# jsourati/nn-active-learning

Hardware: AMD Instinct MI355X
Metric: patches/sec Fisher-scored (32^3, 2-class) (higher is better)
Workload: dtype f32 (fp32 operands split into 16-bit pieces on the 16-bit MFMA, fp32 accumulate: fp16 pairs - 22-23 bits kept per operand, three products - in the conv under the head (forward + backward), in dec1's forward launch and in the other backward launches; bf16 triples - all 24 bits, exact, six products -

## Files before the change

### nn-active-learning_amd/csrc/alq_internal.h

```cpp
#pragma once
#include <hip/hip_runtime.h>

#include <cstdint>
#include <cstdio>
#include <memory>
#include <string>
#include <vector>

#include "alq.h"

namespace alq {

void set_error(const char *fmt, ...);

#define ALQ_HIP(expr)                                                                     \
    do {                                                                                  \
        hipError_t e_ = (expr);                                                           \
        if (e_ != hipSuccess) {                                                           \
            ::alq::set_error("%s:%d: %s -> %s", __FILE__, __LINE__, #expr,               \
                             hipGetErrorString(e_));                                      \
            return ALQ_EHIP;                                                              \
        }                                                                                 \
    } while (0)

// ... 182 lines not shown
    int *d_tdesc = nullptr, *d_sdesc = nullptr;
};

struct Igemm2Fuse {
    const float *mask = nullptr;
    int mask_cs = 0, mask_c0 = 0, mask_from = 0;
    int mask_to = 1 << 30;
    float *osumA = nullptr, *osumB = nullptr;
    int split = 0;
    int store_from = 0;
    int mask_split = 0;
    long long mask_delta = 0;
    const unsigned char *mask_bits = nullptr;
    unsigned char *sign_out = nullptr;
    const unsigned *in_bits = nullptr;
    const float *in_vec = nullptr;
    float in_vec_amax = 0.f;
    const unsigned *in_vec16 = nullptr;
    unsigned *out_amax = nullptr;
    int amax_from = 0;
    const unsigned *in_amax = nullptr, *in_amax2 = nullptr;
    float in_bound = 0.f;
    const float *fc_W = nullptr;
    long long fc_F = 0;
    float *fc_part = nullptr;
    unsigned *fc_bits = nullptr;
    unsigned *flip_cnt = nullptr, *flip_list = nullptr;
    int flip_cap = 0;
    float flip_l1 = 0.f;
    bool flip_bias_nonzero = false;
};

extern unsigned long long *g_igemm2_dbg;
constexpr int ALQ_NKNOBS = 9;
extern int g_dbg_knobs[ALQ_NKNOBS];
extern int g_dcp_last_form;
extern int g_no_f16x2;
extern int g_no_fixed;
extern int g_no_xcd_order;
int igemm2_build_plan(const IgemmPlan &p1, Igemm2Plan *p2);
void igemm2_pack_weights(Igemm2Plan *p2, const std::vector<float> &Bmat);
int igemm2_launch(alq_ctx *ctx, const Igemm2Plan &plan, const View &in, const View &out, const float *bias,
                  int relu, int accumulate, int N, int prof_cls, const Igemm2Fuse *fuse);

struct Igemm3Plan {
    bool ok = false;
    bool wres = false;
    int NTW = 1;
    int wgs_per_cu = 1;
    size_t lds_bytes = 0;
    std::vector<unsigned short> h_W;
    void *d_W = nullptr;
    std::vector<unsigned short> h_W16;
    void *d_W16 = nullptr;
    int w16_exp = 0;
};
int igemm3_build_plan(const Igemm2Plan &p2, Igemm3Plan *p3);
void igemm3_pack_weights(const Igemm2Plan &p2, Igemm3Plan *p3, const std::vector<float> &Bmat);
void igemm3_pack_weights_f16(const Igemm2Plan &p2, Igemm3Plan *p3, const std::vector<float> &Bmat);
int igemm3_launch(alq_ctx *ctx, const Igemm2Plan &p2, const Igemm3Plan &plan, const View &in, const View &out,
                  const float *bias, int relu, int accumulate, int N, int prof_cls, const Igemm2Fuse *fuse);

struct Igemm4Args {
    const float *in;
    float *out;
    const void *W;
    const float *bias;
// ... 103 lines not shown
void c3d_bwd_pack(C3dPlan *plan, const std::vector<float> &Bmat_fwd );
void c3d_presplit_vec(const float *v, long long F, int e, std::vector<unsigned short> *out);
int c3d_bwd_launch(alq_ctx *ctx, const C3dPlan &plan, int N, const unsigned char *bits, const void *vec16, int e_in, const unsigned char *maskA,
                   float *dB, float *sumA, float *sumB, int rows_per_wave = 8);

struct T3dPlan {
    bool ok = false;
    int kind = 0;
    int w_exp = 0;
    double flops_per_patch = 0;
    std::vector<unsigned short> h_W;
    void *d_W = nullptr;
};
int t3d_build(const View &in, const View &out, const int k[3], const int lo[3], const int s[3], T3dPlan *fwd, T3dPlan *bwd);
void t3d_fwd_pack(T3dPlan *plan, const float *W );
void t3d_bwd_pack(T3dPlan *plan, const float *W);
void t3d8_fwd_pack(T3dPlan *plan, const float *W );
void t3d8_bwd_pack(T3dPlan *plan, const float *W );
int t3d8_bwd_launch(alq_ctx *ctx, const T3dPlan &plan, const View &dout, const View &din, int N, float in_bound, const unsigned char *mask_bits, float *dsum);
int t3d_fwd_launch(alq_ctx *ctx, const T3dPlan &plan, const View &in, const View &out, const float *bias, int N, float *osum, unsigned *out_amax);
int t3d_bwd_launch(alq_ctx *ctx, const T3dPlan &plan, const View &dout, const View &din, int N, float in_bound, const unsigned char *mask_bits,
                   float *dsum);

struct E3dPlan {
    bool ok = false;
    int w_exp = 0;
    double flops_per_patch = 0;
    std::vector<unsigned short> h_Whi, h_Wlo;
    void *d_Whi = nullptr, *d_Wlo = nullptr;
};
int e3d_build(const View &in, const View &out, const int k[3], const int lo[3], const int s[3], E3dPlan *plan);
void e3d_pack(E3dPlan *plan, const float *W );
int e3d_bwd_launch(alq_ctx *ctx, const E3dPlan &plan, int N, const float *skip, const float *dpool, const unsigned char *am2, const unsigned char *sg2,
                   const unsigned char *am1, const unsigned char *sg1, float *dsum2, float *dsum1, float in_bound);

struct D3dPlan {
    bool ok = false;
    int w_exp = 0;
    double flops_per_patch = 0;
    std::vector<unsigned short> h_Whi, h_Wlo;
    void *d_Whi = nullptr, *d_Wlo = nullptr;
    std::vector<unsigned short> h_Bhi, h_Blo;
    void *d_Bhi = nullptr, *d_Blo = nullptr;
};
void d3d_bwd_pack(D3dPlan *plan, const float *W);
int d3d_bwd_launch(alq_ctx *ctx, const D3dPlan &plan, int N, const float *dout, float in_bound, float *dinA, float *dinB, float *sumB);
int d3d_build(const View &in, const View &out, const int k[3], const int lo[3], const int s[3], D3dPlan *plan);
void d3d_pack(D3dPlan *plan, const float *W );
int d3d_fwd_launch(alq_ctx *ctx, const D3dPlan &plan, int N, const float *inA, const float *inB, const unsigned *amaxA, const unsigned *amaxB,
                   const float *bias, int relu, float *out, unsigned char *sg, float *osum);

struct F3dPlan {
    bool ok = false;
    int w_exp = 0;
    double flops_per_patch = 0;
    std::vector<unsigned short> h_Whi, h_Wlo;
    void *d_Whi = nullptr, *d_Wlo = nullptr;
};
int f3d_build(const View &in, const View &out, const int k[3], const int lo[3], const int s[3], F3dPlan *plan);
void f3d_pack(F3dPlan *plan, const float *W );
int f3d_fwd_launch(alq_ctx *ctx, const F3dPlan &plan, int N, const float *in, const unsigned *amax, const float *bias, float *out, unsigned char *sg,
                   float *osum, float *pout, unsigned char *parg, float *posum);

struct DirectArgs {
    const float *in;
    float *out;
    const float *W;
// ... 199 lines not shown
```

### nn-active-learning_amd/csrc/e3d.hip

```cpp
#include "alq_internal.h"

#include <algorithm>
#include <cmath>
#include <cstdlib>
#include <cstring>
#include <vector>

namespace alq {

typedef float f32x4 __attribute__((ext_vector_type(4)));
typedef float f32x2 __attribute__((ext_vector_type(2)));
typedef int i32x4 __attribute__((ext_vector_type(4)));
typedef int i32x2 __attribute__((ext_vector_type(2)));
typedef _Float16 f16x8 __attribute__((ext_vector_type(8)));
typedef _Float16 f16x2 __attribute__((ext_vector_type(2)));

struct E3Args {
    const float *skip;
    const float *dpool;
    const unsigned char *am2;
    const unsigned char *sg2;
    const unsigned short *Whi;
    const unsigned short *Wlo;
    const unsigned char *am1;
// ... 192 lines not shown
                        const f16x8 wlo = *reinterpret_cast<const f16x8 *>(wl + ((dz * 3 + dy) * 2 + s) * 1024);
                        const f16x8 whi = wh[dz * 3 + dy][s];
                        cl = __builtin_amdgcn_mfma_f32_16x16x32_f16(wlo, xh, cl, 0, 0, 0);
                        cl = __builtin_amdgcn_mfma_f32_16x16x32_f16(whi, xl, cl, 0, 0, 0);
                        c = __builtin_amdgcn_mfma_f32_16x16x32_f16(whi, xh, c, 0, 0, 0);
                    }
                }
            }
            const float r0 = __builtin_fmaf(cl.x, 0x1p-11f, c.x) * a.inv, r1 = __builtin_fmaf(cl.y, 0x1p-11f, c.y) * a.inv;
            const float r2 = __builtin_fmaf(cl.z, 0x1p-11f, c.z) * a.inv, r3 = __builtin_fmaf(cl.w, 0x1p-11f, c.w) * a.inv;
            unsigned m0 = (unsigned)__builtin_amdgcn_sbfe((int)sg1b, 0, 1), m1 = (unsigned)__builtin_amdgcn_sbfe((int)sg1b, 1, 1);
            unsigned m2 = (unsigned)__builtin_amdgcn_sbfe((int)sg1b, 2, 1), m3 = (unsigned)__builtin_amdgcn_sbfe((int)sg1b, 3, 1);
            asm("" : "+v"(m0), "+v"(m1), "+v"(m2), "+v"(m3));
            const float v0 = __builtin_bit_cast(float, __builtin_bit_cast(unsigned, r0) & m0), v1 = __builtin_bit_cast(float, __builtin_bit_cast(unsigned, r1) & m1);
            const float v2 = __builtin_bit_cast(float, __builtin_bit_cast(unsigned, r2) & m2), v3 = __builtin_bit_cast(float, __builtin_bit_cast(unsigned, r3) & m3);
            float sw[8];
#pragma unroll
            for (int w = 0; w < 8; ++w)
                sw[w] = ((((am1w & 255u) == (unsigned)w) ? v0 : 0.f) + ((((am1w >> 8) & 255u) == (unsigned)w) ? v1 : 0.f)) +
                        (((((am1w >> 16) & 255u) == (unsigned)w) ? v2 : 0.f) + (((am1w >> 24) == (unsigned)w) ? v3 : 0.f));
            f32x4 mine;
            {
                const float g0 = __shfl_xor(hi ? sw[0] : sw[4], 16, 64), g1 = __shfl_xor(hi ? sw[1] : sw[5], 16, 64);
                const float g2 = __shfl_xor(hi ? sw[2] : sw[6], 16, 64), g3 = __shfl_xor(hi ? sw[3] : sw[7], 16, 64);
                mine = f32x4{(hi ? sw[4] : sw[0]) + g0, (hi ? sw[5] : sw[1]) + g1, (hi ? sw[6] : sw[2]) + g2, (hi ? sw[7] : sw[3]) + g3};
            }
            const f32x2 n0 = f32x2{old0.x + mine.x, old0.y + mine.y}, n1 = f32x2{old1.x + mine.z, old1.y + mine.w};
            __builtin_amdgcn_raw_buffer_store_b64(__builtin_bit_cast(i32x2, n0), d1_rsrc, (int)(tv ? e_d1 : E3_OOB), (int)d1row, 0);
            __builtin_amdgcn_raw_buffer_store_b64(__builtin_bit_cast(i32x2, n1), d1_rsrc, (int)(tv ? e_d1 + 128u : E3_OOB), (int)d1row, 0);
        }
    }
}

int e3d_build(const View &in, const View &out, const int k[3], const int lo[3], const int s[3], E3dPlan *plan) {
    plan->ok = false;
    if (getenv("ALQ_NO_E3D")) return ALQ_OK;
    if (!(k[0] == 3 && k[1] == 3 && k[2] == 3 && s[0] == 1 && s[1] == 1 && s[2] == 1 && lo[0] == 1 && lo[1] == 1 && lo[2] == 1)) return ALQ_OK;
    if (!(in.D == 16 && in.H == 16 && in.W == 16 && out.D == 16 && out.H == 16 && out.W == 16 && in.C == 8 && out.C == 16 && in.split == 0 && out.split == 0)) return ALQ_OK;
    plan->flops_per_patch = 2.0 * 27 * 8 * 16 * 4096.0;
    plan->ok = true;
    return ALQ_OK;
}

void e3d_pack(E3dPlan *plan, const float *W) {
    float amax = 0.f;
    for (size_t i = 0; i < (size_t)27 * 8 * 16; ++i) amax = std::max(amax, std::fabs(W[i]));
    int ex = 0;
    if (amax > 0.f) (void)std::frexp(amax, &ex);
    plan->w_exp = 14 - ex;
    plan->h_Whi.assign((size_t)9 * 2 * 64 * 8, 0);
    plan->h_Wlo.assign((size_t)9 * 2 * 64 * 8, 0);
    for (int dz = 0; dz < 3; ++dz)
        for (int dy = 0; dy < 3; ++dy)
            for (int s = 0; s < 2; ++s)
                for (int lane = 0; lane < 64; ++lane) {
                    const int r = lane & 15, kg = lane >> 4, px = r >> 3, ci = r & 7, q = 2 * s + (kg >> 1);
                    const int tz = 2 - dz, ty = 2 - dy, tx = 2 - q + px;
                    for (int c = 0; c < 8; ++c) {
                        const int co = 8 * (kg & 1) + c;
                        const float w = (tx >= 0 && tx <= 2) ? W[((size_t)((tz * 3 + ty) * 3 + tx) * 8 + ci) * 16 + co] : 0.f;
                        const float ws = std::ldexp(w, plan->w_exp);
                        const _Float16 h = (_Float16)ws;
                        const _Float16 l = (_Float16)std::ldexp(ws - (float)h, 11);
                        unsigned short hb, lb;
                        std::memcpy(&hb, &h, 2);
                        std::memcpy(&lb, &l, 2);
                        const size_t o = ((size_t)((dz * 3 + dy) * 2 + s) * 64 + lane) * 8 + c;
                        plan->h_Whi[o] = hb;
                        plan->h_Wlo[o] = lb;
                    }
                }
}

int e3d_bwd_launch(alq_ctx *ctx, const E3dPlan &plan, int N, const float *skip, const float *dpool, const unsigned char *am2, const unsigned char *sg2,
                   const unsigned char *am1, const unsigned char *sg1, float *dsum2, float *dsum1, float in_bound) {
    ALQ_REQUIRE(plan.ok && plan.d_Whi && plan.d_Wlo, ALQ_EINVAL, "e3d: weights not set");
    ALQ_REQUIRE(skip && dpool && am2 && sg2 && am1 && sg1 && dsum2 && dsum1 && in_bound > 0.f, ALQ_EINVAL, "e3d: missing argument");
    ALQ_REQUIRE(N < 4096, ALQ_EUNSUPPORTED, "e3d: 32-bit byte offsets hold fewer than 4096 patches per pass");
    if (N <= 0) return ALQ_OK;
    int ex = 0;
    (void)std::frexp(in_bound, &ex);
    const int e_in = 14 - ex;
    E3Args a;
    a.skip = skip; a.dpool = dpool; a.am2 = am2; a.sg2 = sg2; a.Whi = reinterpret_cast<const unsigned short *>(plan.d_Whi);
    a.Wlo = reinterpret_cast<const unsigned short *>(plan.d_Wlo); a.am1 = am1; a.sg1 = sg1; a.dsum2 = dsum2; a.dsum1 = dsum1;
    a.scale = std::ldexp(1.f, e_in); a.inv = std::ldexp(1.f, -(e_in + plan.w_exp)); a.N = N;
    const int cus = ctx->num_cus;
    long long g = std::min<long long>(2LL * cus, (long long)N * 4);
    g = std::max<long long>(8, (g + 7) / 8 * 8);
    const size_t lds = E3_WLO + E3_STRIP + E3_SINK;
    ALQ_HIP(hipFuncSetAttribute(reinterpret_cast<const void *>(e3d_bwd_kernel), hipFuncAttributeMaxDynamicSharedMemorySize, (int)lds));
    ProfScope ps(ctx, PROF_IGEMM_F16, plan.flops_per_patch * N);
    hipLaunchKernelGGL(e3d_bwd_kernel, dim3((unsigned)g), dim3(256), lds, ctx->stream, a);
    ALQ_HIP(hipGetLastError());
    return ALQ_OK;
}

}
```

### nn-active-learning_amd/csrc/igemm2.hip

```cpp
#include "alq_internal.h"

#include <algorithm>
#include <cmath>
#include <cstring>

namespace alq {

typedef float f32x4 __attribute__((ext_vector_type(4)));
typedef float f32x2 __attribute__((ext_vector_type(2)));

#ifdef ALQ_STAMPS
#define STAMP(var) asm volatile("s_memtime %0\n\ts_waitcnt lgkmcnt(0)" : "=s"(var)::"memory")
#define PHASE_END(idx)                         \
    do {                                       \
        unsigned long long t_now_;             \
        STAMP(t_now_);                         \
        ph[idx] += t_now_ - t_last;            \
        t_last = t_now_;                       \
    } while (0)
#else
#define PHASE_END(idx) do {} while (0)
#endif

constexpr int I2_CBP = 12;
// ... 451 lines not shown
    }
    p2->NTW = p1.NTW;
    p2->wres = wres;
    p2->lds_bytes = lds;
    int max_wgs = 2;
    if (const char *e = getenv("ALQ_MAX_WGS")) max_wgs = atoi(e);
    p2->wgs_per_cu = std::max<int>(1, std::min<int>(max_wgs, (int)((160 * 1024) / (lds + 512))));
    p2->flops_per_patch = p1.flops_per_patch;
    p2->ok = true;
    return ALQ_OK;
}

void igemm2_pack_weights(Igemm2Plan *p2, const std::vector<float> &Bmat) {
    const Igemm2Args &a = p2->a;
    const int NTW = p2->NTW, Ci = a.Ci, Co = a.Co;
    p2->h_W.assign((size_t)a.nchunks * a.ntaps * NTW * 128, 0.f);
    for (int ch = 0; ch < a.nchunks; ++ch)
        for (int tp = 0; tp < a.ntaps; ++tp)
            for (int nt = 0; nt < NTW; ++nt)
                for (int lane = 0; lane < 64; ++lane)
                    for (int s = 0; s < 2; ++s) {
                        const int c = ch * 8 + 2 * (lane >> 4) + s;
                        const int co = nt * 16 + (lane & 15);
                        if (co < Co)
                            p2->h_W[((((size_t)ch * a.ntaps + tp) * NTW + nt) * 64 + lane) * 2 + s] =
                                Bmat[((size_t)tp * Ci + c) * Co + co];
                    }
}

unsigned long long *g_igemm2_dbg = nullptr;
int g_no_f16x2 = 0;
int g_no_xcd_order = 0;
int g_no_fixed = 0;
int g_dbg_knobs[ALQ_NKNOBS] = {0, 0, 0, 0, 0, 0, 0, 0, 0};

template <int NTW, bool WRES, int GEO, bool SUMS>
static int launch2_s(alq_ctx *ctx, const Igemm2Plan &plan, const Igemm2Args &a, unsigned grid) {
    auto kfn = igemm2_kernel<NTW, WRES, GEO, SUMS>;
    if (plan.lds_bytes > 64 * 1024)
        ALQ_HIP(hipFuncSetAttribute(reinterpret_cast<const void *>(kfn), hipFuncAttributeMaxDynamicSharedMemorySize,
                                    (int)plan.lds_bytes));
    hipLaunchKernelGGL(kfn, dim3(grid), dim3(256), plan.lds_bytes, ctx->stream, a);
    ALQ_HIP(hipGetLastError());
    return ALQ_OK;
}

template <int NTW, bool WRES, int GEO>
static int launch2_t(alq_ctx *ctx, const Igemm2Plan &plan, const Igemm2Args &a, unsigned grid) {
    return (a.osumA || a.osumB) ? launch2_s<NTW, WRES, GEO, true>(ctx, plan, a, grid)
                                : launch2_s<NTW, WRES, GEO, false>(ctx, plan, a, grid);
}

int igemm2_launch(alq_ctx *ctx, const Igemm2Plan &plan, const View &in, const View &out, const float *bias, int relu,
                  int accumulate, int N, int prof_cls, const Igemm2Fuse *fuse) {
    Igemm2Args a = plan.a;
    ALQ_REQUIRE(in.C == a.Ci && in.D == a.ID && in.H == a.IH && in.W == a.IW, ALQ_EINVAL,
                "igemm2: input view does not match plan");
    ALQ_REQUIRE(out.C == a.Co && out.D == a.OD && out.H == a.OH && out.W == a.OW, ALQ_EINVAL,
                "igemm2: output view does not match plan");
    ALQ_REQUIRE(plan.d_W != nullptr, ALQ_EINVAL, "igemm2: weights not set");
    ALQ_REQUIRE((long long)N * in.vox() * in.cs < (1LL << 29) && (long long)N * out.vox() * out.cs < (1LL << 29),
                ALQ_EUNSUPPORTED, "igemm2: tensor exceeds the 32-bit byte-offset range (lower the batch)");
    ALQ_REQUIRE(in.cs % 4 == 0 && in.c0 % 4 == 0 && out.cs % 4 == 0 && out.c0 % 4 == 0, ALQ_EUNSUPPORTED,
                "igemm2: channel slice not 16-byte aligned");
    if (fuse) ALQ_REQUIRE(fuse->split % 4 == 0 && fuse->mask_cs % 4 == 0 && fuse->mask_c0 % 4 == 0 && fuse->mask_from % 4 == 0, ALQ_EUNSUPPORTED,
                          "igemm2: fused epilogue needs 4-channel aligned slices");
    a.in = in.p; a.in_cs = in.cs; a.in_c0 = in.c0;
// ... 43 lines not shown
```

### nn-active-learning_amd/csrc/model.hip

```cpp
#include <algorithm>
#include <cmath>
#include <cstdarg>
#include <cstring>
#include <string>
#include <memory>

#include "alq_internal.h"

namespace alq {

static thread_local char g_err[1024] = "";
void set_error(const char *fmt, ...) {
    va_list ap;
    va_start(ap, fmt);
    vsnprintf(g_err, sizeof(g_err), fmt, ap);
    va_end(ap);
}

int gather_normalize_impl(alq_ctx *, const void *const *, int, int, const int64_t[3], const int64_t[3],
                          const int64_t *, int64_t, const int32_t[3], const double *, int, int, void *);
int score_entropy_impl(alq_ctx *, const float *, int64_t, double *, float *);
int synth_impl(alq_ctx *, uint64_t, int64_t, int64_t, int64_t, float *);
int gather_rows_impl(alq_ctx *, const float *, const int64_t *, int64_t, int64_t, float *);
int debug_view_copy(alq_ctx *, const View &, int, float *);
// ... 81 lines not shown
    int max_batch = 0;
    bool last_call_fisher = false;
    bool last_head_fused = false;
    unsigned *amax_a = nullptr, *amax_b = nullptr, *amax_tiles = nullptr;
    unsigned *flip_cnt = nullptr, *flip_list = nullptr;
    int flip_cap = 0;
    unsigned *bound_all = nullptr;
    unsigned *in_amax = nullptr;
    bool v3_fwd_f16 = false;
    unsigned *flip_overflow = nullptr;
    int no_flipfix = 0;
    size_t amax_tiles_len = 0;
    int in_dims[4] = {1, 1, 1, 1};
    int nclass = 0;
    int L = 0;
    std::vector<Layer> layers;
    std::vector<void *> allocs;
    float *logits = nullptr, *dlogits = nullptr, *post = nullptr;
    double *S = nullptr, *sizes = nullptr, *Apart = nullptr;
    double *Spart = nullptr;
    int *nslab = nullptr;
    int nslab_max = 1;
    float *wg_partial = nullptr;
    size_t wg_partial_len = 0;
    double *gn_partial = nullptr;
    size_t gn_partial_len = 0;
    double *df_scratch = nullptr;
    double *ls_part = nullptr;
    std::vector<int> ls_nslab;
    int ls_nslab_max = 0;
    int last_lsum = 0;
    float *x_stage = nullptr;
    int64_t epp = 0;
    int knobs[ALQ_NKNOBS] = {0, 0, 0, 0, 0, 0, 0, 0, 0};
    int no_f16x2 = 0;
    int no_xcd_order = 0;
    int requested_batch = 0;
    int no_bound16 = 0;
    int no_fixed = 0;
    int no_presplit = 0;
    int no_signs = 0;
    int no_signs0 = 0;
    int f16_fwd_mask = -1;
    int f16_fwd_derived = 0;
    int no_f16_derived = 0;
    float *d_bound_L = nullptr, *d_bound_B = nullptr;
    int *d_bound_src = nullptr;
    int no_light_kernels = 0;
    int no_c3d = 0;
    int c3_bwd_rows = 8;
    bool last_c3 = false;
    bool last_c3_bwd = false;
    int no_e3d = 0;
    int last_e3b = 0;
    int no_d3d = 0;
    int last_d3f = 0;
    int no_f3d = 0, last_f3f = 0;
    int no_d3b = 0, last_d3b = 0;
    int no_t3d = 0;
    int last_dcp = 0;
    int last_t3f = 0, last_t3b = 0;
    bool last_f16_derived = false;
    int64_t host_pack_elems = 0;
    void *d_wscal = nullptr;
    bool hv_ready = false;
    double *hv_part = nullptr;
    double *hv_p64 = nullptr;

    template <typename T>
    int dalloc(T **p, size_t count) {
        void *q = nullptr;
        const size_t bytes = std::max<size_t>(count * sizeof(T), 256);
        if (hipMalloc(&q, bytes) != hipSuccess) {
            set_error("hipMalloc of %zu bytes failed", bytes);
            return ALQ_ENOMEM;
        }
        allocs.push_back(q);
        *p = reinterpret_cast<T *>(q);
        return ALQ_OK;
    }
};

int alq_ctx::prof_begin(int cls, hipEvent_t *e0, hipEvent_t *e1) {
    ProfSlot &s = prof[cls];
    auto get = [&](hipEvent_t *ev) -> int {
        if (!s.pool.empty()) {
            *ev = s.pool.back();
// ... 15 lines not shown
}

int alq_ctx::prof_collect() {
    ALQ_HIP(hipStreamSynchronize(stream));
    for (int c = 0; c < PROF_NUM; ++c) {
        ProfSlot &s = prof[c];
        for (auto &pr : s.pending) {
            float ms = 0.f;
            ALQ_HIP(hipEventElapsedTime(&ms, pr.first, pr.second));
            s.ms += ms;
            s.pool.push_back(pr.first);
            s.pool.push_back(pr.second);
        }
        s.pending.clear();
    }
    return ALQ_OK;
}

static int upload1(alq_model *m, IgemmPlan *p) {
    if (!p->d_W) ALQ_TRY(m->dalloc(&p->d_W, p->h_W.size()));
    ALQ_HIP(hipMemcpyAsync(p->d_W, p->h_W.data(), p->h_W.size() * sizeof(float), hipMemcpyHostToDevice,
                           m->ctx->stream));
    if (p->smallc) {
        if (!p->d_koff) ALQ_TRY(m->dalloc(&p->d_koff, p->h_koff.size()));
        ALQ_HIP(hipMemcpyAsync(p->d_koff, p->h_koff.data(), p->h_koff.size() * sizeof(int),
                               hipMemcpyHostToDevice, m->ctx->stream));
    }
    ALQ_HIP(hipStreamSynchronize(m->ctx->stream));
    std::vector<float>().swap(p->h_W);
    return ALQ_OK;
}

static bool g_use_v2 = true;
static int g_knob_override[ALQ_NKNOBS] = {-1, -1, -1, -1, -1, -1, -1, -1, -1};

static void apply_knobs(const alq_model *m) {
    for (int k = 0; k < ALQ_NKNOBS; ++k) g_dbg_knobs[k] = g_knob_override[k] >= 0 ? g_knob_override[k] : m->knobs[k];
    g_no_f16x2 = m->no_f16x2;
    g_no_xcd_order = m->no_xcd_order;
    g_no_fixed = m->no_fixed;
}

static int gemm_build(const ConvDesc &d, int max_batch, Gemm *g, const G4Geom *g4 = nullptr) {
    ALQ_TRY(igemm_build_plan(d, max_batch, &g->p1));
    if (g4 && !getenv("ALQ_DISABLE_V4")) {
        G4Geom gg = *g4;
        gg.flops_per_patch = g->p1.flops_per_patch;
        ALQ_TRY(igemm4_build_plan(gg, max_batch, &g->p4));
    }
    ALQ_TRY(igemm2_build_plan(g->p1, &g->p2));
    ALQ_TRY(direct_build_plan(g->p1, &g->pd));
    if (!g_use_v2) { g->p2.ok = false; g->pd.ok = false; }
    ALQ_TRY(igemm3_build_plan(g->p2, &g->p3));
    if (d.ID == 1 && d.IH == 1 && d.IW == 1 && d.tz.size() == 1 && d.sm == 1 && d.so == 1 && !getenv("ALQ_NO_FCGEMM"))
        ALQ_TRY(fcgemm_build_plan(d.Ci, d.Co, &g->pfc));
    if (const char *e = getenv("ALQ_DISABLE_V3")) { if (e[0] == '1') g->p3.ok = false; }
    return ALQ_OK;
}

static int set4(alq_model *m, Igemm4Plan *p4, const std::vector<float> &Bmat) {
    igemm4_pack_weights(p4, Bmat);
    hipStream_t st = m->ctx->stream;
    if (!p4->d_tdesc) {
        ALQ_TRY(m->dalloc(&p4->d_tdesc, p4->h_tdesc.size()));
        ALQ_TRY(m->dalloc(&p4->d_sdesc, p4->h_sdesc.size()));
        ALQ_TRY(m->dalloc(&p4->d_pdesc, p4->h_pdesc.size()));
        ALQ_TRY(m->dalloc(&p4->d_ttab, p4->h_ttab.size()));
// ... 916 lines not shown
static int run_backward_main(alq_model *m, const float *d_x, int N) {
    alq_ctx *ctx = m->ctx;
    const int nl = (int)m->layers.size();
    ALQ_REQUIRE(m->nclass == 2, ALQ_EUNSUPPORTED, "Fisher scoring is binary (PW_NNAL.py:766), got %d classes", m->nclass);
    ALQ_TRY(k_fill_unit_cotangent(ctx, m->dlogits, N));
    for (Layer &l : m->layers) { l.delta_ready = false; l.dsum_partial = false; l.dout_bits = nullptr; l.dout_vec = nullptr; l.dout_vec16 = nullptr; l.dout_vec16c = nullptr; l.dout_amax = nullptr; }
    m->last_c3_bwd = false;
    m->last_t3b = 0;
    const bool v4_on = !g_dbg_knobs[4] && !g_dbg_knobs[5];
    {
        for (Layer &l : m->layers) l.dout_bound = 0.f;
        m->layers[nl - 1].dout_bound = 1.f;
        for (int i = nl - 1; i >= 1; --i) {
            const Layer &ly = m->layers[i];
            double inb = ly.dout_bound;
            if (ly.spec.type == ALQ_FC)
                inb = (ly.spec.cout == 2 && ly.fc_wv_amax > 0.f && i == nl - 1) ? (double)ly.fc_wv_amax : (i < nl - 1 ? ly.bwd_l1 * ly.dout_bound : 0.0);
            else if (ly.spec.type != ALQ_POOL) inb = ly.bwd_l1 * ly.dout_bound;
            if (!(inb > 0.0) || ly.dout_bound <= 0.f) inb = 0.0;
            auto add = [&](Layer &p) { p.dout_bound = (p.dout_bound < 0.f || inb <= 0.0) ? -1.f : p.dout_bound + (float)(inb * (1.0 + 1e-6)); };
            add(m->layers[i - 1]);
            if (ly.spec.skip_src >= 0) add(m->layers[ly.spec.skip_src]);
        }
    }
    auto pool_first_ok = [&](const Layer &pl, const Layer &src) {
        return pl.spec.type == ALQ_POOL && src.pidx == 0 && src.spec.type != ALQ_FC && pl.spec.k[1] == 2 && pl.spec.k[2] == 2 &&
               (pl.spec.k[0] == 1 || pl.spec.k[0] == 2) && pl.lo[0] == 0 && pl.lo[1] == 0 && pl.lo[2] == 0 &&
               src.out.D == pl.out.D * pl.spec.k[0] && src.out.H == pl.out.H * 2 && src.out.W == pl.out.W * 2 &&
               (pl.out.C == 4 || pl.out.C == 8 || pl.out.C == 16) && ((pl.dout.cs | pl.dout.c0 | pl.out.cs | pl.out.c0) & 3) == 0 &&
               src.spec.relu && !g_dbg_knobs[6];
    };
    int e3_conv = -1;
    m->last_e3b = 0;
    m->last_d3b = 0;
    for (int i = nl - 1; i >= 0; --i) {
        Layer &ly = m->layers[i];
        const bool prev_is_src = (i > 0 && m->layers[i - 1].out_is_skip_src && ly.spec.skip_src < 0);
        if (ly.spec.type == ALQ_POOL && i >= 3 && !m->no_e3d && v4_on && !g_no_f16x2 && !m->no_bound16 && !m->no_signs && !g_dbg_knobs[2] && !g_dbg_knobs[6]) {
            Layer &cv = m->layers[i - 1], &p1 = m->layers[i - 2], &c0 = m->layers[i - 3];
            const bool geo = cv.spec.type == ALQ_CONV && cv.e3b.ok && cv.e3b.d_Whi && cv.spec.relu && cv.signs_ready && cv.out.sg && prev_is_src &&
                             p1.spec.type == ALQ_POOL && pool_first_ok(p1, c0) && c0.dsum_partial && p1.signs_ready && p1.out.sg && p1.spec.k[0] == 2 &&
                             ly.spec.k[0] == 2 && ly.spec.k[1] == 2 && ly.spec.k[2] == 2 && ly.lo[0] == 0 && ly.lo[1] == 0 && ly.lo[2] == 0 &&
                             ly.dout.D == 8 && ly.dout.H == 8 && ly.dout.W == 8 && ly.dout.C == 16 && ly.dout.cs == 16 && ly.dout.c0 == 0 && !ly.dout.split &&
                             cv.dout.cs == 16 && cv.dout.c0 == 0 && !cv.dout.split && cv.out.cs == 16 && cv.out.c0 == 0 && p1.out.cs == 8 && p1.out.c0 == 0 &&
                             p1.out.C == 8 && c0.out.D == 32 && cv.dout_bound > 0.f && cv.dsum && c0.dsum;
            if (geo) {
                ALQ_TRY(e3d_bwd_launch(ctx, cv.e3b, N, cv.dout.p, ly.dout.p, ly.argmax, cv.out.sg, p1.argmax, p1.out.sg, cv.dsum, c0.dsum, cv.dout_bound));
                cv.delta_ready = true;
                c0.delta_ready = true;
                e3_conv = i - 1;
                m->last_e3b = 1;
                continue;
            }
        }
        if (e3_conv >= 0 && i == e3_conv - 1) continue;
        Layer *prev = i > 0 ? &m->layers[i - 1] : nullptr;
        const bool prev_param = prev && prev->pidx >= 0 && prev->spec.type != ALQ_FC;
        if (ly.spec.type == ALQ_POOL && prev_param && pool_first_ok(ly, *prev) && (prev->dsum_partial || !prev_is_src)) {
            ALQ_TRY(k_pool_bwd_first(ctx, ly.dout, ly.out, ly.argmax, ly.spec.k, prev->out.D, prev->out.H, prev->out.W, N,
                                     prev->dsum, prev->dsum_partial ? 1 : 0, ly.signs_ready ? 1 : 0));
            prev->delta_ready = true;
            continue;
        }
        if (ly.spec.type == ALQ_POOL) {
            bool fused = false;
            ALQ_TRY(k_pool_bwd(ctx, ly.dout, ly.din, ly.argmax, ly.spec.k, ly.lo, N, prev_is_src ? 1 : 0,
                               (prev_param && prev->spec.relu) ? &prev->out : nullptr, prev_param ? prev->dsum : nullptr,
                               &fused, !(prev_param && prev->pidx == 0),
                               (prev_param && prev->signs_ready) ? 1 : 0));
            if (prev_param && fused) prev->delta_ready = true;
            continue;
        }
        const bool isfc = ly.spec.type == ALQ_FC;
        if (!ly.delta_ready) {
            View dv = isfc ? flat_view(ly.dout) : ly.dout;
            View av = isfc ? flat_view(ly.out) : ly.out;
            ALQ_TRY(k_mask_chansum(ctx, dv, ly.spec.relu ? &av : nullptr, ly.dsum, N));
        }
        const float *as1 = ly.asum, *as2 = nullptr;
        if (!isfc) {
// ... 793 lines not shown
}

int alq_ctx_synchronize(alq_ctx *ctx) {
    ALQ_REQUIRE(ctx != nullptr, ALQ_EINVAL, "null ctx");
    ALQ_HIP(hipStreamSynchronize(ctx->stream));
    return ALQ_OK;
}

int alq_model_create(alq_ctx *ctx, const alq_layer_t *layers, int n_layers, const int32_t in_dims[4],
                     int max_batch, alq_model **out) {
    ALQ_REQUIRE(ctx && layers && in_dims && out, ALQ_EINVAL, "alq_model_create: null argument");
    ALQ_REQUIRE(n_layers >= 1 && n_layers <= 64 && max_batch >= 1, ALQ_EINVAL, "alq_model_create: bad sizes");
    ALQ_HIP(hipSetDevice(ctx->device));
    alq_model *m = new alq_model();
    m->ctx = ctx;
    m->max_batch = max_batch;
    {
        const char *e = getenv("ALQ_DISABLE_V2");
        g_use_v2 = !(e && e[0] == '1');
        m->no_f16x2 = getenv("ALQ_NO_F16X2") != nullptr;
        m->no_xcd_order = getenv("ALQ_NO_XCD_ORDER") != nullptr;
        m->no_fixed = getenv("ALQ_NO_FIXED") != nullptr;
        m->no_bound16 = getenv("ALQ_NO_BOUND16") != nullptr;
        m->no_flipfix = getenv("ALQ_NO_FLIPFIX") != nullptr;
        m->no_presplit = getenv("ALQ_NO_PRESPLIT") != nullptr;
        m->no_c3d = getenv("ALQ_NO_C3D") != nullptr;
        m->no_light_kernels = getenv("ALQ_NO_LIGHT_KERNELS") != nullptr;
        { const char *e = getenv("ALQ_C3D_BWD_ROWS"); m->c3_bwd_rows = (e && atoi(e) == 4) ? 4 : ((e && atoi(e) == 8) ? 8 : 7); }
        m->no_signs = getenv("ALQ_NO_SIGNS") != nullptr;
        m->no_signs0 = getenv("ALQ_NO_SIGNS0") != nullptr;
        if (const char *f = getenv("ALQ_F16_FWD_MASK")) m->f16_fwd_mask = atoi(f);
        m->no_t3d = getenv("ALQ_NO_T3D") ? 1 : 0;
        m->no_e3d = getenv("ALQ_NO_E3D") ? 1 : 0;
        m->no_d3d = getenv("ALQ_NO_D3D") ? 1 : 0;
        m->no_f3d = getenv("ALQ_NO_F3D") ? 1 : 0;
        m->no_d3b = getenv("ALQ_NO_D3D_BWD") ? 1 : 0;
        {
            const char *e = getenv("ALQ_F16_DERIVED"), *n = getenv("ALQ_NO_F16_DERIVED");
            m->no_f16_derived = ((e && atoi(e) == 0) || (n && atoi(n) == 1)) ? 1 : 0;
        }
        static const char *names[ALQ_NKNOBS] = {"ALQ_DEBUG_REPEAT", "ALQ_DEBUG_FLAGS", "ALQ_NO_BWD_FUSE", "ALQ_NO_FWD_FUSE", "ALQ_NO_V3", "ALQ_NO_V4",
                                                "ALQ_NO_POOL_FIRST", "ALQ_NO_CONV_POOL", "ALQ_DCP_NARROW"};
        for (int k = 0; k < ALQ_NKNOBS; ++k) {
            const char *v = getenv(names[k]);
            if (v) m->knobs[k] = atoi(v);
        }
    }
    for (int i = 0; i < 4; ++i) m->in_dims[i] = in_dims[i];
    m->epp = (int64_t)in_dims[0] * in_dims[1] * in_dims[2] * in_dims[3];
    const int rc = build_model(m, layers, n_layers);
    if (rc != ALQ_OK) {
        alq_model_destroy(m);
        return rc;
    }
    if (const char *t = getenv("ALQ_G4_TUNE")) {
        std::string all(t);
        size_t pos = 0;
        while (pos < all.size()) {
            size_t end = all.find(';', pos);
            if (end == std::string::npos) end = all.size();
            const std::string item = all.substr(pos, end - pos);
            pos = end + 1;
            if (item.size() < 3 || (item[0] != 'f' && item[0] != 'b')) continue;
            const size_t colon = item.find(':');
            if (colon == std::string::npos) continue;
            const int li = atoi(item.substr(1, colon - 1).c_str());
            if (li < 0 || li >= (int)m->layers.size()) continue;
            Layer &ly = m->layers[li];
            Igemm4Plan *pl = item[0] == 'b' ? &ly.bwd.p4 : (ly.spec.type == ALQ_CONVT ? &ly.fwd_all : (ly.fwd.empty() ? nullptr : &ly.fwd[0].p4));
            if (!pl) continue;
            const size_t fi = item.find("fic="), ei = item.find("epi=");
            if (fi != std::string::npos) pl->tune_fic = atoi(item.c_str() + fi + 4);
            if (ei != std::string::npos) pl->tune_epi = atoi(item.c_str() + ei + 4);
        }
    }
// ... 609 lines not shown
            const View &v = ly.out;
            ALQ_REQUIRE(v.sg && ly.signs_ready && ((v.C | v.cs | v.c0) & 3) == 0 && ((int64_t)N * v.vox() * v.cs) % 16 == 0, ALQ_EUNSUPPORTED,
                        "layer %d: no sign field of its output in the last pass", layer_idx);
            if (elems_out) *elems_out = (int64_t)N * v.vox() * v.cs / 16;
            ALQ_HIP(hipMemcpyAsync(d_out, v.sg, (size_t)N * v.vox() * v.cs / 4, hipMemcpyDeviceToDevice, m->ctx->stream));
            return ALQ_OK;
        }
        ALQ_REQUIRE(ly.spec.type == ALQ_POOL && ly.argmax && ((int64_t)N * ly.out.vox() * ly.out.C) % 4 == 0, ALQ_EUNSUPPORTED, "layer %d has no arg-max field", layer_idx);
        if (elems_out) *elems_out = (int64_t)N * ly.out.vox() * ly.out.C / 4;
        ALQ_HIP(hipMemcpyAsync(d_out, ly.argmax, (size_t)N * ly.out.vox() * ly.out.C, hipMemcpyDeviceToDevice, m->ctx->stream));
        return ALQ_OK;
    }
    if (what == 0 || what == 1) {
        const Layer &head = m->layers.back();
        ALQ_REQUIRE(!(layer_idx + 2 == (int)m->layers.size() && head.spec.type == ALQ_FC &&
                      (what == 0 ? m->last_head_fused
                                 : (m->last_call_fisher && head.fc_maskbits != nullptr && !g_dbg_knobs[4] && !g_dbg_knobs[5]))),
                    ALQ_EUNSUPPORTED, "layer %d: this tensor is not materialised in a Fisher pass (fc head fused into the layer: "
                    "create the model under ALQ_NO_FC_BITS=1 to keep it)", layer_idx);
        const View &v = what == 0 ? ly.out : ly.dout;
        if (elems_out) *elems_out = (int64_t)N * v.elems();
        return debug_view_copy(m->ctx, v, N, d_out);
    }
    ALQ_REQUIRE(ly.pidx >= 0 && (what == 2 || what == 3), ALQ_EINVAL, "layer has no channel-sum fields");
    const bool isfc = ly.spec.type == ALQ_FC;
    const int64_t e = (int64_t)N * (isfc ? 1 : (what == 2 ? ly.in.vox() : ly.out.vox()));
    if (elems_out) *elems_out = e;
    ALQ_HIP(hipMemcpyAsync(d_out, what == 2 ? ly.asum : ly.dsum, e * sizeof(float), hipMemcpyDeviceToDevice,
                           m->ctx->stream));
    return ALQ_OK;
}

int alq_model_engine_info(alq_model *m, int what) {
    ALQ_REQUIRE(m && ((what >= 0 && what <= 3) || (what >= 5 && what <= 16)), ALQ_EINVAL, "alq_model_engine_info: bad argument");
    if (what == 16) return m->last_dcp;
    if (what == 15) return m->last_lsum;
    if (what == 14) return m->host_pack_elems > 0x7fffffffll ? 0x7fffffff : (int)m->host_pack_elems;
    if (what == 13) return m->last_c3_bwd ? m->c3_bwd_rows : 0;
    if (what == 6) return m->last_f16_derived ? 1 : 0;
    if (what == 7) return m->last_t3f;
    if (what == 8) return m->last_t3b;
    if (what == 12) return m->last_f3f;
    if (what == 11) return m->last_d3b;
    if (what == 10) return m->last_d3f;
    if (what == 9) return m->last_e3b;
    ALQ_HIP(hipSetDevice(m->ctx->device));
    if (what == 0) return c3d_subnormals_ok(m->ctx);
    if (what == 1) return m->last_c3 ? 1 : 0;
    if (what == 2) return m->last_c3_bwd ? 1 : 0;
    if (what == 5) {
        if (!m->flip_overflow) return 0;
        unsigned h = 0;
        ALQ_HIP(hipMemcpyAsync(&h, m->flip_overflow, sizeof(unsigned), hipMemcpyDeviceToHost, m->ctx->stream));
        ALQ_HIP(hipStreamSynchronize(m->ctx->stream));
        return h > 0x7fffffffu ? 0x7fffffff : (int)h;
    }
    for (const Layer &ly : m->layers)
        if (ly.c3f.ok) return ly.c3f.oneacc;
    return 0;
}

int alq_debug_set(int key, int value) {
    ALQ_REQUIRE(key >= 0 && key < ALQ_NKNOBS, ALQ_EINVAL, "alq_debug_set: bad key");
    g_knob_override[key] = value > 0 ? value : -1;
    g_dbg_knobs[key] = value;
    return ALQ_OK;
}
// ... 15 lines not shown
```

Baseline: 274,100.

## Add plane-sweep e3d backward kernel with a rotating LDS z-plane ring

Adds a new e3d backward kernel, now the default, in which each block sweeps the 16 z-planes of whole patches. A 4-slot LDS ring holds the fp16 hi/lo gradient images of consecutive planes, so each plane's image is built once and reused by the three dz taps instead of rebuilding halos per row strip. Loads for later planes are prefetched in registers while the current plane runs its MFMAs. The grid drops to about one block per CU (capped by patches), which may cut parallelism for small batches. The older row kernel stays behind ALQ_E3D_ROWS=1.

```diff
diff --git a/nn-active-learning_amd/csrc/alq_internal.h b/nn-active-learning_amd/csrc/alq_internal.h
--- a/nn-active-learning_amd/csrc/alq_internal.h
+++ b/nn-active-learning_amd/csrc/alq_internal.h
@@ -238,7 +238,7 @@
 };
 
 extern unsigned long long *g_igemm2_dbg;
-constexpr int ALQ_NKNOBS = 9;
+constexpr int ALQ_NKNOBS = 10;
 extern int g_dbg_knobs[ALQ_NKNOBS];
 extern int g_dcp_last_form;
 extern int g_no_f16x2;
@@ -408,7 +408,8 @@
 int e3d_build(const View &in, const View &out, const int k[3], const int lo[3], const int s[3], E3dPlan *plan);
 void e3d_pack(E3dPlan *plan, const float *W );
 int e3d_bwd_launch(alq_ctx *ctx, const E3dPlan &plan, int N, const float *skip, const float *dpool, const unsigned char *am2, const unsigned char *sg2,
-                   const unsigned char *am1, const unsigned char *sg1, float *dsum2, float *dsum1, float in_bound);
+                   const unsigned char *am1, const unsigned char *sg1, float *dsum2, float *dsum1, float in_bound,
+                   bool rows );
 
 struct D3dPlan {
     bool ok = false;
diff --git a/nn-active-learning_amd/csrc/e3d.hip b/nn-active-learning_amd/csrc/e3d.hip
--- a/nn-active-learning_amd/csrc/e3d.hip
+++ b/nn-active-learning_amd/csrc/e3d.hip
@@ -248,6 +248,191 @@
     }
 }
 
+constexpr int E3Z_IMG = 18 * E3_SLOT;
+constexpr int E3Z_ZERO = 4 * E3Z_IMG;
+constexpr int E3Z_SINK = 5 * E3Z_IMG;
+constexpr int E3Z_LDS = E3_WLO + E3Z_SINK + E3_SLOT;
+static_assert(E3Z_IMG % 16 == 0 && E3Z_LDS <= 160 * 1024, "e3d plane sweep: LDS layout");
+
+struct E3ZRowB { f32x4 dp; unsigned am; };
+
+__global__ __launch_bounds__(512) void e3d_bwdz_kernel(const E3Args a) {
+    extern __shared__ __attribute__((aligned(16))) char e3lds[];
+    {
+        const i32x4 *src = reinterpret_cast<const i32x4 *>(a.Wlo);
+        i32x4 *dst = reinterpret_cast<i32x4 *>(e3lds);
+        for (int i = threadIdx.x; i < E3_WLO / 16; i += 512) dst[i] = src[i];
+        for (int i = threadIdx.x; i < (E3Z_LDS - E3_WLO) / 16; i += 512) dst[E3_WLO / 16 + i] = i32x4{0, 0, 0, 0};
+    }
+    __syncthreads();
+    const int lane = threadIdx.x & 63, wave = __builtin_amdgcn_readfirstlane((int)(threadIdx.x >> 6));
+    char *strip = e3lds + E3_WLO;
+    const int n = lane & 15, kg = lane >> 4, ry = n >> 3, j = n & 7;
+    f16x8 wh[9][2];
+#pragma unroll
+    for (int c = 0; c < 9; ++c)
+#pragma unroll
+        for (int s = 0; s < 2; ++s) wh[c][s] = *reinterpret_cast<const f16x8 *>(a.Whi + ((size_t)(c * 2 + s) * 64 + lane) * 8);
+#pragma unroll
+    for (int c = 0; c < 9; ++c)
+#pragma unroll
+        for (int s = 0; s < 2; ++s) asm volatile("" : "+v"(wh[c][s]));
+    const char *wl = e3lds + lane * 16;
+
+    const __amdgpu_buffer_rsrc_t sk_rsrc = e3_rsrc(a.skip, (unsigned long long)a.N * 4096 * 64);
+    const __amdgpu_buffer_rsrc_t dp_rsrc = e3_rsrc(a.dpool, (unsigned long long)a.N * 512 * 64);
+    const __amdgpu_buffer_rsrc_t a2_rsrc = e3_rsrc(a.am2, (unsigned long long)a.N * 512 * 16);
+    const __amdgpu_buffer_rsrc_t s2_rsrc = e3_rsrc(a.sg2, (unsigned long long)a.N * 4096 * 4);
+    const __amdgpu_buffer_rsrc_t a1_rsrc = e3_rsrc(a.am1, (unsigned long long)a.N * 4096 * 8);
+    const __amdgpu_buffer_rsrc_t s1_rsrc = e3_rsrc(a.sg1, (unsigned long long)a.N * 4096 * 2);
+    const __amdgpu_buffer_rsrc_t d2_rsrc = e3_rsrc(a.dsum2, (unsigned long long)a.N * 4096 * 4);
+    const __amdgpu_buffer_rsrc_t d1_rsrc = e3_rsrc(a.dsum1, (unsigned long long)a.N * 32768 * 4);
+
+    const int sx = lane >> 2, cq = lane & 3;
+    const int w_off = (sx + 1) * 32 + cq * 8 + (2 * wave + 1) * E3_SLOT;
+    const unsigned ldA = (unsigned)lane * 16u, ldS = (unsigned)lane;
+    const unsigned ldP = (unsigned)(sx >> 1) * 64u + (unsigned)cq * 16u, ldM = (unsigned)(sx >> 1) * 16u + (unsigned)cq * 4u;
+    const unsigned lanepar4 = (unsigned)(sx & 1) * 0x01010101u;
+    const unsigned st2 = cq == 0 ? (unsigned)sx * 4u : E3_OOB;
+    const int f_off = (2 * j + (kg >> 1)) * 32 + (kg & 1) * 16 + (2 * wave + ry) * E3_SLOT;
+    const bool hi = (kg & 1) != 0;
+    const unsigned e_am = (unsigned)(ry * 16 + 2 * j + (kg >> 1)) * 8u + (unsigned)(kg & 1) * 4u;
+    const unsigned e_sg = (unsigned)(ry * 16 + 2 * j + (kg >> 1)) * 2u + (unsigned)(kg & 1);
+    const unsigned e_d1 = (unsigned)(hi ? 32 * 128 : 0) + (unsigned)(2 * ry) * 128u + (unsigned)(2 * (2 * j + (kg >> 1))) * 4u;
+
+    const int G = (int)gridDim.x, b0 = (int)blockIdx.x;
+    const int nunits = a.N > b0 ? (a.N - b0 + G - 1) / G : 0;
+    const int T = nunits * 16;
+
+    auto plane = [&](int m, int *p, int *z) __attribute__((always_inline)) {
+        const int mc = m < 0 ? 0 : (m < T ? m : T - 1);
+        *p = b0 + (mc >> 4) * G;
+        *z = mc & 15;
+    };
+    auto fetchA = [&](int m, E3RowA *R) __attribute__((always_inline)) {
+        int p, z;
+        plane(m, &p, &z);
+        const unsigned row = ((unsigned)p * 16u + (unsigned)z) * 16u + (unsigned)(2 * wave);
+        const int so_sk = e3_s(row * 1024u), so_sg = e3_s(row * 64u);
+#pragma unroll
+        for (int r = 0; r < 2; ++r) {
+            R[r].sk = __builtin_bit_cast(f32x4, __builtin_amdgcn_raw_buffer_load_b128(sk_rsrc, (int)(ldA + (unsigned)r * 1024u), so_sk, 0));
+            R[r].sg = (unsigned)(unsigned char)__builtin_amdgcn_raw_buffer_load_b8(s2_rsrc, (int)(ldS + (unsigned)r * 64u), so_sg, 0);
+        }
+    };
+    auto fetchB = [&](int m, E3ZRowB *R) __attribute__((always_inline)) {
+        int p, z;
+        plane(m, &p, &z);
+        const unsigned prow = ((unsigned)p * 8u + (unsigned)(z >> 1)) * 8u + (unsigned)wave;
+        R->dp = __builtin_bit_cast(f32x4, __builtin_amdgcn_raw_buffer_load_b128(dp_rsrc, (int)ldP, e3_s(prow * 512u), 0));
+        R->am = (unsigned)__builtin_amdgcn_raw_buffer_load_b32(a2_rsrc, (int)ldM, e3_s(prow * 128u), 0);
+    };
+
+    E3RowA RA[2][2];
+    E3ZRowB RB;
+    RB.dp = f32x4{0.f, 0.f, 0.f, 0.f}; RB.am = 0u;
+#pragma unroll
+    for (int i = 0; i < 2; ++i)
+#pragma unroll
+        for (int b = 0; b < 2; ++b) { RA[b][i].sk = f32x4{0.f, 0.f, 0.f, 0.f}; RA[b][i].sg = 0u; }
+
+    if (T > 0)
+    for (int s0 = -2; s0 < T + 2; s0 += 2) {
+#pragma unroll
+        for (int b = 0; b < 2; ++b) {
+            __builtin_amdgcn_sched_barrier(0);
+            const int s = s0 + b;
+            const bool live = s0 >= 0 && s < T;
+            const bool tv = s >= 2;
+            int p, z, po, zo;
+            plane(s, &p, &z);
+            plane(s - 2, &po, &zo);
+            asm volatile("s_waitcnt lgkmcnt(0)\n\ts_barrier" ::: "memory");
+            const unsigned trow = ((unsigned)po * 16u + (unsigned)zo) * 16u + (unsigned)(2 * wave);
+            const unsigned am1w = (unsigned)__builtin_amdgcn_raw_buffer_load_b32(a1_rsrc, (int)e_am, e3_s(trow * 128u), 0);
+            const unsigned sg1b = (unsigned)(unsigned char)__builtin_amdgcn_raw_buffer_load_b8(s1_rsrc, (int)e_sg, e3_s(trow * 32u), 0);
+            const unsigned d1row = (unsigned)e3_s((((unsigned)po * 32u + (unsigned)(2 * zo)) * 32u + (unsigned)(4 * wave)) * 128u);
+            const f32x2 old0 = __builtin_bit_cast(f32x2, __builtin_amdgcn_raw_buffer_load_b64(d1_rsrc, (int)e_d1, (int)d1row, 0));
+            const f32x2 old1 = __builtin_bit_cast(f32x2, __builtin_amdgcn_raw_buffer_load_b64(d1_rsrc, (int)(e_d1 + 128u), (int)d1row, 0));
+            const unsigned srow = ((unsigned)p * 16u + (unsigned)z) * 16u + (unsigned)(2 * wave);
+            const int so_d2 = e3_s(srow * 64u);
+            char *img = strip + e3_s(live ? (unsigned)(s & 3) * (unsigned)E3Z_IMG : (unsigned)(E3Z_SINK - (2 * wave + 1) * E3_SLOT)) + w_off;
+            const float scr = a.scale;
+#pragma unroll
+            for (int r = 0; r < 2; ++r) {
+                const E3RowA &ra = RA[b][r];
+                const unsigned x4 = RB.am ^ (lanepar4 ^ ((unsigned)((((z & 1) * 2 + r) * 2)) * 0x01010101u));
+                float g0 = ra.sk.x + (((x4 & 0xffu) == 0u) ? RB.dp.x : 0.f);
+                float g1 = ra.sk.y + (((x4 & 0xff00u) == 0u) ? RB.dp.y : 0.f);
+                float g2 = ra.sk.z + (((x4 & 0xff0000u) == 0u) ? RB.dp.z : 0.f);
+                float g3 = ra.sk.w + (((x4 & 0xff000000u) == 0u) ? RB.dp.w : 0.f);
+                unsigned k0 = (unsigned)__builtin_amdgcn_sbfe((int)ra.sg, 0, 1), k1 = (unsigned)__builtin_amdgcn_sbfe((int)ra.sg, 1, 1);
+                unsigned k2 = (unsigned)__builtin_amdgcn_sbfe((int)ra.sg, 2, 1), k3 = (unsigned)__builtin_amdgcn_sbfe((int)ra.sg, 3, 1);
+                asm("" : "+v"(k0), "+v"(k1), "+v"(k2), "+v"(k3));
+                g0 = __builtin_bit_cast(float, __builtin_bit_cast(unsigned, g0) & k0); g1 = __builtin_bit_cast(float, __builtin_bit_cast(unsigned, g1) & k1);
+                g2 = __builtin_bit_cast(float, __builtin_bit_cast(unsigned, g2) & k2); g3 = __builtin_bit_cast(float, __builtin_bit_cast(unsigned, g3) & k3);
+                {
+                    float s_ = (g0 + g1) + (g2 + g3);
+                    s_ += __builtin_bit_cast(float, __builtin_amdgcn_mov_dpp(__builtin_bit_cast(int, s_), 0xB1, 0xf, 0xf, true));
+                    s_ += __builtin_bit_cast(float, __builtin_amdgcn_mov_dpp(__builtin_bit_cast(int, s_), 0x4E, 0xf, 0xf, true));
+                    __builtin_amdgcn_raw_buffer_store_b32(__builtin_bit_cast(int, s_), d2_rsrc, (int)(live ? st2 + (unsigned)r * 64u : E3_OOB), so_d2, 0);
+                }
+                const float x0 = g0 * scr, x1 = g1 * scr, x2 = g2 * scr, x3 = g3 * scr;
+                const f16x2 h01 = __builtin_convertvector(f32x2{x0, x1}, f16x2), h23 = __builtin_convertvector(f32x2{x2, x3}, f16x2);
+                const float sc11 = scr * 2048.f;
+                const f16x2 l01 = __builtin_convertvector(f32x2{__builtin_fmaf((float)h01.x, -2048.f, g0 * sc11), __builtin_fmaf((float)h01.y, -2048.f, g1 * sc11)}, f16x2);
+                const f16x2 l23 = __builtin_convertvector(f32x2{__builtin_fmaf((float)h23.x, -2048.f, g2 * sc11), __builtin_fmaf((float)h23.y, -2048.f, g3 * sc11)}, f16x2);
+                char *dst = img + (live ? r * E3_SLOT : 0);
+                *reinterpret_cast<i32x2 *>(dst) = i32x2{__builtin_bit_cast(int, h01), __builtin_bit_cast(int, h23)};
+                *reinterpret_cast<i32x2 *>(dst + E3_ROWB) = i32x2{__builtin_bit_cast(int, l01), __builtin_bit_cast(int, l23)};
+            }
+            fetchB(s + 1, &RB);
+            fetchA(s + 2, RA[b]);
+            const int io[3] = {e3_s(zo == 0 ? (unsigned)E3Z_ZERO : (unsigned)((s + 1) & 3) * (unsigned)E3Z_IMG), e3_s((unsigned)((s + 2) & 3) * (unsigned)E3Z_IMG),
+                               e3_s(zo == 15 ? (unsigned)E3Z_ZERO : (unsigned)((s + 3) & 3) * (unsigned)E3Z_IMG)};
+            f32x4 c = f32x4{0.f, 0.f, 0.f, 0.f}, cl = f32x4{0.f, 0.f, 0.f, 0.f};
+#pragma unroll
+            for (int dy = 0; dy < 3; ++dy) {
+#pragma unroll
+                for (int dz = 0; dz < 3; ++dz) {
+                    const char *src = strip + io[dz] + f_off + dy * E3_SLOT;
+#pragma unroll
+                    for (int s2 = 0; s2 < 2; ++s2) {
+                        const f16x8 xh = *reinterpret_cast<const f16x8 *>(src + s2 * 64);
+                        const f16x8 xl = *reinterpret_cast<const f16x8 *>(src + s2 * 64 + E3_ROWB);
+                        const f16x8 wlo = *reinterpret_cast<const f16x8 *>(wl + ((dz * 3 + dy) * 2 + s2) * 1024);
+                        const f16x8 whi = wh[dz * 3 + dy][s2];
+                        cl = __builtin_amdgcn_mfma_f32_16x16x32_f16(wlo, xh, cl, 0, 0, 0);
+                        cl = __builtin_amdgcn_mfma_f32_16x16x32_f16(whi, xl, cl, 0, 0, 0);
+                        c = __builtin_amdgcn_mfma_f32_16x16x32_f16(whi, xh, c, 0, 0, 0);
+                    }
+                }
+            }
+            const float r0 = __builtin_fmaf(cl.x, 0x1p-11f, c.x) * a.inv, r1 = __builtin_fmaf(cl.y, 0x1p-11f, c.y) * a.inv;
+            const float r2 = __builtin_fmaf(cl.z, 0x1p-11f, c.z) * a.inv, r3 = __builtin_fmaf(cl.w, 0x1p-11f, c.w) * a.inv;
+            unsigned m0 = (unsigned)__builtin_amdgcn_sbfe((int)sg1b, 0, 1), m1 = (unsigned)__builtin_amdgcn_sbfe((int)sg1b, 1, 1);
+            unsigned m2 = (unsigned)__builtin_amdgcn_sbfe((int)sg1b, 2, 1), m3 = (unsigned)__builtin_amdgcn_sbfe((int)sg1b, 3, 1);
+            asm("" : "+v"(m0), "+v"(m1), "+v"(m2), "+v"(m3));
+            const float v0 = __builtin_bit_cast(float, __builtin_bit_cast(unsigned, r0) & m0), v1 = __builtin_bit_cast(float, __builtin_bit_cast(unsigned, r1) & m1);
+            const float v2 = __builtin_bit_cast(float, __builtin_bit_cast(unsigned, r2) & m2), v3 = __builtin_bit_cast(float, __builtin_bit_cast(unsigned, r3) & m3);
+            float sw[8];
+#pragma unroll
+            for (int w = 0; w < 8; ++w)
+                sw[w] = ((((am1w & 255u) == (unsigned)w) ? v0 : 0.f) + ((((am1w >> 8) & 255u) == (unsigned)w) ? v1 : 0.f)) +
+                        (((((am1w >> 16) & 255u) == (unsigned)w) ? v2 : 0.f) + (((am1w >> 24) == (unsigned)w) ? v3 : 0.f));
+            f32x4 mine;
+            {
+                const float g0 = __shfl_xor(hi ? sw[0] : sw[4], 16, 64), g1 = __shfl_xor(hi ? sw[1] : sw[5], 16, 64);
+                const float g2 = __shfl_xor(hi ? sw[2] : sw[6], 16, 64), g3 = __shfl_xor(hi ? sw[3] : sw[7], 16, 64);
+                mine = f32x4{(hi ? sw[4] : sw[0]) + g0, (hi ? sw[5] : sw[1]) + g1, (hi ? sw[6] : sw[2]) + g2, (hi ? sw[7] : sw[3]) + g3};
+            }
+            const f32x2 n0 = f32x2{old0.x + mine.x, old0.y + mine.y}, n1 = f32x2{old1.x + mine.z, old1.y + mine.w};
+            __builtin_amdgcn_raw_buffer_store_b64(__builtin_bit_cast(i32x2, n0), d1_rsrc, (int)(tv ? e_d1 : E3_OOB), (int)d1row, 0);
+            __builtin_amdgcn_raw_buffer_store_b64(__builtin_bit_cast(i32x2, n1), d1_rsrc, (int)(tv ? e_d1 + 128u : E3_OOB), (int)d1row, 0);
+        }
+    }
+}
+
 int e3d_build(const View &in, const View &out, const int k[3], const int lo[3], const int s[3], E3dPlan *plan) {
     plan->ok = false;
     if (getenv("ALQ_NO_E3D")) return ALQ_OK;
@@ -289,7 +474,7 @@
 }
 
 int e3d_bwd_launch(alq_ctx *ctx, const E3dPlan &plan, int N, const float *skip, const float *dpool, const unsigned char *am2, const unsigned char *sg2,
-                   const unsigned char *am1, const unsigned char *sg1, float *dsum2, float *dsum1, float in_bound) {
+                   const unsigned char *am1, const unsigned char *sg1, float *dsum2, float *dsum1, float in_bound, bool rows) {
     ALQ_REQUIRE(plan.ok && plan.d_Whi && plan.d_Wlo, ALQ_EINVAL, "e3d: weights not set");
     ALQ_REQUIRE(skip && dpool && am2 && sg2 && am1 && sg1 && dsum2 && dsum1 && in_bound > 0.f, ALQ_EINVAL, "e3d: missing argument");
     ALQ_REQUIRE(N < 4096, ALQ_EUNSUPPORTED, "e3d: 32-bit byte offsets hold fewer than 4096 patches per pass");
@@ -302,6 +487,16 @@
     a.Wlo = reinterpret_cast<const unsigned short *>(plan.d_Wlo); a.am1 = am1; a.sg1 = sg1; a.dsum2 = dsum2; a.dsum1 = dsum1;
     a.scale = std::ldexp(1.f, e_in); a.inv = std::ldexp(1.f, -(e_in + plan.w_exp)); a.N = N;
     const int cus = ctx->num_cus;
+    if (!rows) {
+        long long g = std::min<long long>(cus, N);
+        g = std::max<long long>(8, (g + 7) / 8 * 8);
+        if (g_dbg_knobs[9] > 0) g = std::min<long long>(g, g_dbg_knobs[9]);
+        ALQ_HIP(hipFuncSetAttribute(reinterpret_cast<const void *>(e3d_bwdz_kernel), hipFuncAttributeMaxDynamicSharedMemorySize, E3Z_LDS));
+        ProfScope ps(ctx, PROF_IGEMM_F16, plan.flops_per_patch * N);
+        hipLaunchKernelGGL(e3d_bwdz_kernel, dim3((unsigned)g), dim3(512), (size_t)E3Z_LDS, ctx->stream, a);
+        ALQ_HIP(hipGetLastError());
+        return ALQ_OK;
+    }
     long long g = std::min<long long>(2LL * cus, (long long)N * 4);
     g = std::max<long long>(8, (g + 7) / 8 * 8);
     const size_t lds = E3_WLO + E3_STRIP + E3_SINK;
diff --git a/nn-active-learning_amd/csrc/igemm2.hip b/nn-active-learning_amd/csrc/igemm2.hip
--- a/nn-active-learning_amd/csrc/igemm2.hip
+++ b/nn-active-learning_amd/csrc/igemm2.hip
@@ -507,7 +507,7 @@
 int g_no_f16x2 = 0;
 int g_no_xcd_order = 0;
 int g_no_fixed = 0;
-int g_dbg_knobs[ALQ_NKNOBS] = {0, 0, 0, 0, 0, 0, 0, 0, 0};
+int g_dbg_knobs[ALQ_NKNOBS] = {0, 0, 0, 0, 0, 0, 0, 0, 0, 0};
 
 template <int NTW, bool WRES, int GEO, bool SUMS>
 static int launch2_s(alq_ctx *ctx, const Igemm2Plan &plan, const Igemm2Args &a, unsigned grid) {
diff --git a/nn-active-learning_amd/csrc/model.hip b/nn-active-learning_amd/csrc/model.hip
--- a/nn-active-learning_amd/csrc/model.hip
+++ b/nn-active-learning_amd/csrc/model.hip
@@ -137,7 +137,7 @@
     int last_lsum = 0;
     float *x_stage = nullptr;
     int64_t epp = 0;
-    int knobs[ALQ_NKNOBS] = {0, 0, 0, 0, 0, 0, 0, 0, 0};
+    int knobs[ALQ_NKNOBS] = {0, 0, 0, 0, 0, 0, 0, 0, 0, 0};
     int no_f16x2 = 0;
     int no_xcd_order = 0;
     int requested_batch = 0;
@@ -158,6 +158,8 @@
     bool last_c3_bwd = false;
     int no_e3d = 0;
     int last_e3b = 0;
+    int e3d_rows = 0;
+    int last_e3b_form = 0;
     int no_d3d = 0;
     int last_d3f = 0;
     int no_f3d = 0, last_f3f = 0;
@@ -239,7 +241,7 @@
 }
 
 static bool g_use_v2 = true;
-static int g_knob_override[ALQ_NKNOBS] = {-1, -1, -1, -1, -1, -1, -1, -1, -1};
+static int g_knob_override[ALQ_NKNOBS] = {-1, -1, -1, -1, -1, -1, -1, -1, -1, -1};
 
 static void apply_knobs(const alq_model *m) {
     for (int k = 0; k < ALQ_NKNOBS; ++k) g_dbg_knobs[k] = g_knob_override[k] >= 0 ? g_knob_override[k] : m->knobs[k];
@@ -1222,6 +1224,7 @@
     };
     int e3_conv = -1;
     m->last_e3b = 0;
+    m->last_e3b_form = 0;
     m->last_d3b = 0;
     for (int i = nl - 1; i >= 0; --i) {
         Layer &ly = m->layers[i];
@@ -1235,7 +1238,8 @@
                              cv.dout.cs == 16 && cv.dout.c0 == 0 && !cv.dout.split && cv.out.cs == 16 && cv.out.c0 == 0 && p1.out.cs == 8 && p1.out.c0 == 0 &&
                              p1.out.C == 8 && c0.out.D == 32 && cv.dout_bound > 0.f && cv.dsum && c0.dsum;
             if (geo) {
-                ALQ_TRY(e3d_bwd_launch(ctx, cv.e3b, N, cv.dout.p, ly.dout.p, ly.argmax, cv.out.sg, p1.argmax, p1.out.sg, cv.dsum, c0.dsum, cv.dout_bound));
+                ALQ_TRY(e3d_bwd_launch(ctx, cv.e3b, N, cv.dout.p, ly.dout.p, ly.argmax, cv.out.sg, p1.argmax, p1.out.sg, cv.dsum, c0.dsum, cv.dout_bound, m->e3d_rows != 0));
+                m->last_e3b_form = m->e3d_rows ? 1 : 2;
                 cv.delta_ready = true;
                 c0.delta_ready = true;
                 e3_conv = i - 1;
@@ -2095,6 +2099,7 @@
         if (const char *f = getenv("ALQ_F16_FWD_MASK")) m->f16_fwd_mask = atoi(f);
         m->no_t3d = getenv("ALQ_NO_T3D") ? 1 : 0;
         m->no_e3d = getenv("ALQ_NO_E3D") ? 1 : 0;
+        { const char *e = getenv("ALQ_E3D_ROWS"); m->e3d_rows = (e && atoi(e) == 1) ? 1 : 0; }
         m->no_d3d = getenv("ALQ_NO_D3D") ? 1 : 0;
         m->no_f3d = getenv("ALQ_NO_F3D") ? 1 : 0;
         m->no_d3b = getenv("ALQ_NO_D3D_BWD") ? 1 : 0;
@@ -2103,7 +2108,7 @@
             m->no_f16_derived = ((e && atoi(e) == 0) || (n && atoi(n) == 1)) ? 1 : 0;
         }
         static const char *names[ALQ_NKNOBS] = {"ALQ_DEBUG_REPEAT", "ALQ_DEBUG_FLAGS", "ALQ_NO_BWD_FUSE", "ALQ_NO_FWD_FUSE", "ALQ_NO_V3", "ALQ_NO_V4",
-                                                "ALQ_NO_POOL_FIRST", "ALQ_NO_CONV_POOL", "ALQ_DCP_NARROW"};
+                                                "ALQ_NO_POOL_FIRST", "ALQ_NO_CONV_POOL", "ALQ_DCP_NARROW", "ALQ_E3D_GRID_CAP"};
         for (int k = 0; k < ALQ_NKNOBS; ++k) {
             const char *v = getenv(names[k]);
             if (v) m->knobs[k] = atoi(v);
@@ -2779,7 +2784,8 @@
 }
 
 int alq_model_engine_info(alq_model *m, int what) {
-    ALQ_REQUIRE(m && ((what >= 0 && what <= 3) || (what >= 5 && what <= 16)), ALQ_EINVAL, "alq_model_engine_info: bad argument");
+    ALQ_REQUIRE(m && ((what >= 0 && what <= 3) || (what >= 5 && what <= 17)), ALQ_EINVAL, "alq_model_engine_info: bad argument");
+    if (what == 17) return m->last_e3b_form;
     if (what == 16) return m->last_dcp;
     if (what == 15) return m->last_lsum;
     if (what == 14) return m->host_pack_elems > 0x7fffffffll ? 0x7fffffff : (int)m->host_pack_elems;
```

Result: faster. 278,100, median of 6 (+1.5%).
